# cvjena/ITAL

Measured on AMD Instinct MI355X. Metric: MI-scored candidates/sec per fetch_unlabelled(k) round, higher is better.
Workload: dtype f64; 1 GPU; USPS-shaped synthetic 9298x256, k=4, perfect user, full 2^t enumeration, fetch_unlabelled + update per step; n=9298, d=256, k=4, parallelism=candidate rows sharded over 1 GPU(s), 1 record all-gather per greedy step

## Files before the change

ital_amd/_lib.py:

```python
import ctypes
import os

HERE = os.path.dirname(os.path.abspath(__file__))
LIB_PATH = os.environ.get("ITAL_HIP_LIB", os.path.join(HERE, "libital_hip.so"))

c_void_p, c_int, c_int64, c_double = ctypes.c_void_p, ctypes.c_int, ctypes.c_int64, ctypes.c_double

ITAL_MAX_T = 8
ITAL_REC_HEADER = 10
ITAL_JUMP_BITS = 48
ITAL_GENERIC_MAX_DIM = 20
ITAL_GENERIC_MAX_REL = 16
ITAL_GENERIC_MAX_CALLS = 1 << 22
ITAL_TOPK_MAX = 4096
ITAL_ROUND_MAX_CAND = 1 << 21


class ItalBatch(ctypes.Structure):
    _fields_ = [("kmax", c_int), ("ldx", c_int), ("ldw", c_int), ("bidx", c_void_p), ("bgpos", c_void_p),
                ("bsort", c_void_p), ("bmu", c_void_p), ("sig", c_void_p), ("XB", c_void_p), ("XBn", c_void_p),
                ("VB", c_void_p)]


class ItalLabelBatch(ctypes.Structure):
# ... 264 lines not shown


ROWS_SIGNATURES = dict(
    [(name + "_t", _typed(SIGNATURES[name])) for name in
     ("ital_rbf_cols", "ital_cross_cov_cols", "ital_whiten_append", "ital_gp_append", "ital_score_step", "ital_fetch_round",
      "ital_select_local", "ital_select_fused", "ital_gather_block")] +
    [("ital_whiten_rows_t", _typed(REWHITEN_SIGNATURES["ital_whiten_rows"])),
     ("ital_ingest_rows_t", (c_int, [c_void_p, c_int, c_int64, c_int, c_int64, c_void_p, c_int, c_void_p, c_void_p, c_int64,
                                     c_void_p]))])


COMPACT_SIGNATURES = {
    "ital_compact_rows": (c_int, [c_void_p, c_void_p, c_int64, c_int, c_int, c_void_p, c_int64, c_void_p, c_void_p, c_void_p,
                                  c_void_p]),
    "ital_compact_cols": (c_int, [c_void_p, c_int64, c_int, c_void_p, c_void_p, c_int64, c_void_p, c_int64, c_void_p, c_int64,
                                  c_int, c_void_p, c_void_p, c_void_p, c_void_p]),
}


CTX_LIVE_SIGNATURES = {
    "ital_ctx_reserve": (c_int, [c_void_p, c_int, c_void_p]),
    "ital_ctx_add_rows": (c_int, [c_void_p, c_void_p, c_int64, c_int, c_void_p]),
    "ital_ctx_remove_rows": (c_int, [c_void_p, c_void_p, c_int64, c_void_p, c_void_p]),
    "ital_ctx_set_params": (c_int, [c_void_p, c_double, c_double, c_double, c_void_p]),
    "ital_ctx_evidence": (c_int, [c_void_p, c_void_p, c_int, c_void_p, c_void_p, c_void_p]),
}


COSINE_SIGNATURES = {
    "ital_cosine_min": (c_int, [c_void_p, c_int, c_void_p, c_int64, c_int, c_void_p, c_void_p, c_int, c_int, c_void_p, c_void_p]),
}


class ItalHipError(RuntimeError):
    pass


def load(path=LIB_PATH):
    if not os.path.exists(path):
        raise ImportError(
            f"{path} not found: build it with `python -m ital_amd.build` (hipcc, gfx950). "
            "ital_amd has no CPU fallback.")
    try:
        import torch
    except ImportError:
        pass
    lib = ctypes.CDLL(path)
    for name, (res, args) in list(SIGNATURES.items()) + list(CTX_SIGNATURES.items()) + list(DENSE_SIGNATURES.items()) + \
            list(ADAPT_SIGNATURES.items()) + list(REVOKE_SIGNATURES.items()) + list(REWHITEN_SIGNATURES.items()) + \
            list(EVIDENCE_SIGNATURES.items()) + list(INGEST_SIGNATURES.items()) + list(ROWS_SIGNATURES.items()) + \
            list(COMPACT_SIGNATURES.items()) + list(EVIDENCE_GRAD_SIGNATURES.items()) + list(LOO_GRAD_SIGNATURES.items()) + \
            list(CTX_LIVE_SIGNATURES.items()) + list(COSINE_SIGNATURES.items()) + list(INFLUENCE_SIGNATURES.items()) + \
            list(CTX_AUDIT_SIGNATURES.items()):
        fn = getattr(lib, name)
        fn.restype = res
        fn.argtypes = args
    return lib


_lib = None


def lib():
    global _lib
    if _lib is None:
        _lib = load()
    return _lib


def rows_fn(name, xtype):
    if xtype == INGEST_F64:
        return getattr(lib(), name)
    fn = getattr(lib(), name + "_t")
    return lambda *args: fn(*(args[:-1] + (xtype, args[-1])))


def check(rc):
    if rc != 0:
        raise ItalHipError(f"libital_hip: error {rc}: {lib().ital_last_error().decode()}")


def legacy_normals(n_skip, n_out, threads=1):
    import numpy as np
    n_skip, n_out = int(n_skip), int(n_out)
    state = np.random.get_state(legacy=True)
    if state[0] != "MT19937":
# ... 13 lines not shown
```

ital_amd/csrc/score.hip:

```cpp
#include <hip/hip_runtime.h>
#include <stdint.h>

#include <type_traits>

#include "device_math.h"
#include "ital_hip.h"
#include "ital_internal.h"
#include "ital_rows.h"
#include "qmc_common.h"
#include "qmc_exact.h"
#include "qmc_seed.h"
#include "qmc_share.h"
#include "select_common.h"

#ifndef ITAL_QMC_HOTK
#define ITAL_QMC_HOTK 1
#endif
#ifndef ITAL_QMC_MAIN_NH
#define ITAL_QMC_MAIN_NH(T) ((T) == 6 || (T) == 8 ? 2 : 3)
#endif
#ifndef ITAL_QMC_WAVES
#define ITAL_QMC_WAVES(T) ((T) <= 4 || (T) == 6 || (T) == 8 ? 4 : 3)
#endif
#ifndef ITAL_QMC_MAIN_PS
#define ITAL_QMC_MAIN_PS(T) ((T) >= 7)
#endif
#ifndef ITAL_QMC_MAIN_KE6
#define ITAL_QMC_MAIN_KE6(T) ((T) == 8)
#endif
#ifndef ITAL_QMC_MAIN_KEN
#define ITAL_QMC_MAIN_KEN(T) ((T) == 7 ? 2 : -1)
#endif
#ifndef ITAL_QMC_MAIN_KE
#define ITAL_QMC_MAIN_KE(T) 1
#endif
#ifndef ITAL_QMC_MAIN_KS
#define ITAL_QMC_MAIN_KS(T) 0
#endif
#ifndef ITAL_QMC_MAIN_CFL
#define ITAL_QMC_MAIN_CFL(T) ((T) >= 7)
#endif

#ifndef ITAL_QMC_SHARE_LAST
#define ITAL_QMC_SHARE_LAST 1
#endif
#ifndef ITAL_QMC_BATCH_DIV
#define ITAL_QMC_BATCH_DIV 1
#endif
#ifndef ITAL_QMC_BATCH_PHINV
#define ITAL_QMC_BATCH_PHINV(T) ((T) <= 4 ? 3 : 0)
#endif
#ifndef ITAL_QMC_BATCH_PHI
#define ITAL_QMC_BATCH_PHI(T) ((T) <= 4 ? 3 : 0)
#endif
#ifndef ITAL_QMC_SHARE_RECS
#define ITAL_QMC_SHARE_RECS 4
#endif
#ifndef ITAL_QMC_SHARE_VCF
#define ITAL_QMC_SHARE_VCF 3
#endif

namespace ital {

struct ScoreArgs {
    int t;
    int64_t n_cand;
    const int32_t* cand;
    const uint8_t* alive;
    const double* mu;
    const double* s2;
    const double* C;
    int64_t ldc;
    int64_t row_offset;
    int64_t pos_offset;
    const int64_t* gpos;
    ital_batch b;
    double noise, eps;
    int label_mode;
    double* mi;
    int seed[6];
    const long long* jump;
    const long long* jumppat;
    const double* vk;
    int* status;
    SelectTail sel;
};

__device__ __forceinline__ double log_eps(double p, double eps) { return log(p + eps); }

__device__ __forceinline__ void mi_accumulate(double& mi, double pr, double pu, double eps, int mode) {
    double cur = log_eps(pu, eps) - log_eps(pr, eps);
    if (mode == 1) {
// ... 76 lines not shown
        const int64_t pc = (int64_t)blockIdx.x * 32 + threadIdx.x;
        if (pc < a.n_cand && a.alive[pc]) {
            double mi = 0.0;
#pragma unroll
            for (int q = 0; q < 4; q++) mi_accumulate(mi, vals[0][4 * threadIdx.x + q], vals[1][4 * threadIdx.x + q], a.eps, a.label_mode);
            a.mi[pc] = mi;
            c.val = mi;
            c.pos = a.gpos ? a.gpos[pc] : a.pos_offset + pc;
            c.loc = pc;
        }
    }
    if (a.sel.enabled) {
        c = block_best(c, 0);
        select_tail(a.sel, c, blockIdx.x, gridDim.x, true, gridDim.x);
    }
}

template <int T>
struct Qmc {
    static constexpr int NDIM = T - 1;
    static constexpr int NP = NDIM < 10 ? NDIM : 10;
    static constexpr int PRIME = P_TAB[NP - 1];
    static constexpr int NCOV = T * (T + 1) / 2;
    static constexpr int NCOR = T * (T - 1) / 2;
    static constexpr int NPAT = 1 << T;
    static constexpr int NCALLS = 2 << T;
    static constexpr int LAT = 8 * NDIM * 2;
    static constexpr int LATP = 5 * NDIM;
    static constexpr int R_LIM = NCOR, R_META = NCOR + T, R_LAT = NCOR + T + 1;
    static constexpr int REC = R_LAT + LATP;
    static constexpr int SLAB_RAW = NCOV + 2 * T + NDIM;
    static constexpr int SLAB = SLAB_RAW | 1;
    static constexpr int PREP_THREADS = T <= 6 ? 256 : 128;
    static constexpr int NH = ITAL_QMC_MAIN_NH(T);
    static constexpr int BPHI = ITAL_QMC_BATCH_DIV && !ITAL_LATTICE_PHI_CF ? ITAL_QMC_BATCH_PHI(T) : 0;
    static constexpr int BINV = ITAL_QMC_BATCH_DIV ? ITAL_QMC_BATCH_PHINV(T) : 0;
    static constexpr int TAILQ = 128 * NH;
    static constexpr bool PS = ITAL_QMC_MAIN_PS(T), CFL = PS && ITAL_QMC_MAIN_CFL(T);
    static constexpr bool SHARE = ITAL_QMC_SHARE_LAST && ITAL_QMC_HOTK && ITAL_QMC_FLIP && !PS &&
                                  QmcRounds<T, NH>::NCL == 1 && ITAL_QMC_SHARE_RECS * QmcRounds<T, NH>::REST <= 64 &&
                                  NPAT % ITAL_QMC_SHARE_RECS == 0;
    static constexpr int RPW = SHARE ? ITAL_QMC_SHARE_RECS : 1;
    static constexpr int WAVE_DOUBLES = LAT + TAILQ + (CFL ? NCOR + T : 0) + (SHARE ? 64 + 2 * RPW + 6 : 0);
    typedef typename std::conditional<(CFL && ITAL_QMC_MAIN_KS(T)), HotKS,
                typename std::conditional<(ITAL_QMC_MAIN_KEN(T) >= 0), HotKEn<(ITAL_QMC_MAIN_KEN(T) >= 0 ? ITAL_QMC_MAIN_KEN(T) : 0)>,
                typename std::conditional<(ITAL_QMC_MAIN_KE6(T)), HotKE6,
                    typename std::conditional<(ITAL_QMC_MAIN_KE(T)), HotKE, HotK>::type>::type>::type>::type Coef;
    static constexpr int64_t CAND_DOUBLES = (int64_t)NPAT * (REC + 1) + 3;
};
constexpr long long META_EVAL = 1, META_PRIOR_ONE = 2, META_POST_ONE = 4;
constexpr long long META_EXACT = 8;

template <int T>
__device__ void rcswp(int p, int q, double* cov, double* lim, unsigned& infi) {
    double tmp = lim[p]; lim[p] = lim[q]; lim[q] = tmp;
    unsigned bp = (infi >> p) & 1u, bq = (infi >> q) & 1u;
    infi = (infi & ~((1u << p) | (1u << q))) | (bq << p) | (bp << q);
    tmp = cov[pidx(p, p)]; cov[pidx(p, p)] = cov[pidx(q, q)]; cov[pidx(q, q)] = tmp;
    for (int j = 0; j < p; j++) { tmp = cov[pidx(p, j)]; cov[pidx(p, j)] = cov[pidx(q, j)]; cov[pidx(q, j)] = tmp; }
    for (int i = p + 1; i < q; i++) { tmp = cov[pidx(i, p)]; cov[pidx(i, p)] = cov[pidx(q, i)]; cov[pidx(q, i)] = tmp; }
    for (int i = q + 1; i < T; i++) { tmp = cov[pidx(i, p)]; cov[pidx(i, p)] = cov[pidx(i, q)]; cov[pidx(i, q)] = tmp; }
}

template <int T>
__device__ bool covsrt(double* cov, double* lim, double* y, unsigned& infi) {
    const double SQTWPI = 2.506628274631001, EPS = 1e-10;
    bool ok = true;
    for (int i = 0; i < T; i++) {
        double dmin = 0, emin = 1, zmin = 0, cvdiag = 0;
        int jmin = i;
        for (int j = i; j < T; j++) {
            const double cjj = cov[pidx(j, j)];
            if (cjj > EPS) {
                const double sumsq = sqrt_pos(cjj);
                double sum = 0;
// ... 27 lines not shown
        } else {
            ok = false;
            y[i] = 0;
        }
    }
    return ok;
}

template <int T>
__device__ __forceinline__ int early_verdict(const double (&l)[T]) {
    const double thr = 37.0 + 9.0 * sqrt((double)(T - 1));
    bool all_full = true, any_empty = false;
#pragma unroll
    for (int a = 0; a < T; a++) {
        if (l[a] > thr) any_empty = true;
        if (!(l[a] < -thr)) all_full = false;
    }
    return any_empty ? 4 : (all_full ? 2 : 0);
}

__device__ __forceinline__ int64_t list_position(const ScoreArgs& a, int64_t p) { return a.gpos ? a.gpos[p] : a.pos_offset + p; }

__global__ __launch_bounds__(256) void qmc_seed_kernel(SeedArgs s) {
    qmc_seed_body(s, (int64_t)blockIdx.x * blockDim.x + threadIdx.x);
}

static SeedArgs seed_args(const ScoreArgs& a, int ncalls, int64_t slab_lo, int64_t slab_n, int* seeds) {
    SeedArgs s = {a.alive, a.gpos, a.pos_offset, a.b.bgpos, a.t - 1, {a.seed[0], a.seed[1], a.seed[2], a.seed[3], a.seed[4], a.seed[5]},
                  a.jump, ncalls, slab_lo, slab_n, seeds};
    return s;
}

template <int T>
__global__ __launch_bounds__(Qmc<T>::PREP_THREADS) void qmc_prep_kernel(ScoreArgs a, int64_t slab_lo, int64_t slab_n,
                                                                         const int* __restrict__ seeds,
                                                                         double* __restrict__ recs) {
    using Q = Qmc<T>;
    extern __shared__ double lds_all[];
    const int64_t i = (int64_t)blockIdx.x * blockDim.x + threadIdx.x;
    if (i >= slab_n) return;
    const int64_t p = slab_lo + i;
    if (!a.alive[p]) return;
    const int r = blockIdx.y;
    const int row = a.cand[p];
    double* rec = recs + ((int64_t)i * Q::NPAT + r) * Q::REC;

    double mean[T], Sg[T][T];
#pragma unroll
    for (int v = 0; v < T - 1; v++) {
        mean[v] = a.b.bmu[v];
#pragma unroll
        for (int j = 0; j < T - 1; j++) Sg[v][j] = a.b.sig[v * a.b.kmax + j];
        const double c = a.C[(int64_t)v * a.ldc + row];
        Sg[v][T - 1] = c;
        Sg[T - 1][v] = c;
    }
    mean[T - 1] = a.mu[row];
    Sg[T - 1][T - 1] = a.s2[row];
    double sd[T], own[T];
    long long meta = 0;
    {
        double Lc[T][T];
#pragma unroll
        for (int v = 0; v < T; v++)
#pragma unroll
            for (int j = 0; j <= v; j++) {
                double x = Sg[v][j] + (v == j ? a.noise : 0.0);
#pragma unroll
                for (int q = 0; q < j; q++) x -= Lc[v][q] * Lc[j][q];
                Lc[v][j] = (v == j) ? sqrt(x) : x / Lc[j][j];
// ... 73 lines not shown
            if (sat0) verdict = 4;
            else if (sat1) verdict = 2;
            else evaluate = true;
        }
    }
    if (verdict == 2) meta |= META_PRIOR_ONE;
    if (evaluate) {
        meta |= META_EVAL | ((long long)infi << 8);
        const unsigned fl = ITAL_QMC_FLIP ? infi : 0u;
        for (int v = 1; v < T; v++)
            for (int j = 0; j < v; j++)
                rec[v * (v - 1) / 2 + j] = (((fl >> v) ^ (fl >> j)) & 1u) ? -cov[pidx(v, j)] : cov[pidx(v, j)];
        for (int v = 0; v < T; v++) rec[Q::R_LIM + v] = ((fl >> v) & 1u) ? -lim[v] : lim[v];
        const int* sp = seeds + i * 6;
        MrgState sti = {sp[0], sp[1], sp[2], sp[3], sp[4], sp[5]};
        mrg_apply(sti, a.jumppat + (int64_t)r * 18);
        MrgStateF st = mrg_to_f(sti);
        for (int j = 0; j < Q::NDIM; j++) gen[j] = (double)j;
        unsigned int* shifts = reinterpret_cast<unsigned int*>(rec + Q::R_LAT);
        unsigned char* perm = reinterpret_cast<unsigned char*>(rec + Q::R_LAT + 4 * Q::NDIM);
        for (int sft = 0; sft < 8; sft++) {
            for (int j = 1; j <= Q::NDIM - 1; j++) {
                const double u = mrg_next_f(st);
                const int jp = (int)(j + u * (Q::NDIM + 1 - j));
                const double xt = gen[j - 1];
                gen[j - 1] = gen[jp - 1];
                gen[jp - 1] = xt;
            }
            for (int j = 0; j < Q::NDIM; j++) perm[sft * Q::NDIM + j] = (unsigned char)gen[j];
            for (int j = 0; j < Q::NDIM; j++) shifts[sft * Q::NDIM + j] = (unsigned int)mrg_next_z(st);
        }
    }
    rec[Q::R_META] = __longlong_as_double(meta);
}

template <int T>
__device__ __forceinline__ void qmc_main_shared(const uint8_t* __restrict__ alive, int64_t slab_lo, int64_t slab_n,
                                                const double* __restrict__ recs, const double* __restrict__ vk, double eps,
                                                int label_mode, double* __restrict__ terms) {
    using Q = Qmc<T>;
    using R = QmcRounds<T, Q::NH>;
    extern __shared__ double lds_all[];
    const int lane = threadIdx.x & 63;
    const int wid = __builtin_amdgcn_readfirstlane(threadIdx.x >> 6);
    const int64_t item0 = ((int64_t)blockIdx.x * 4 + wid) * Q::RPW;
    const int64_t i = item0 >> T;
    if (i >= slab_n) return;
    if (!alive[slab_lo + i]) return;
    double* lat = lds_all + (size_t)wid * Q::WAVE_DOUBLES;
    double* tailq = lat + Q::LAT;
    int first = -1;
    for (int j = Q::RPW - 1; j >= 0; j--)
        if (__double_as_longlong(uniform_f64(recs[(item0 + j) * Q::REC + Q::R_META])) & META_EVAL) first = j;
    double* lastv = tailq + Q::TAILQ;
    typename Q::Coef kk;
    kk.load();
    if (first >= 0) {
        const int j_own = lane >> 4;
        bool dead = j_own >= Q::RPW;
        if (!dead) dead = !(__double_as_longlong(recs[(item0 + j_own) * Q::REC + Q::R_META]) & META_EVAL);
        const double* rec = recs + (item0 + (dead ? first : j_own)) * Q::REC;
        const unsigned flips = (unsigned)(__double_as_longlong(rec[Q::R_META]) >> 8) & ((1u << T) - 1u);
        double cf[Q::NCOR > 0 ? Q::NCOR : 1], lm[T], xx[Q::NDIM > 0 ? Q::NDIM : 1];
#pragma unroll
        for (int q = 0; q < Q::NCOR; q++) cf[q] = rec[q];
#pragma unroll
        for (int q = 0; q < T; q++) lm[q] = rec[Q::R_LIM + q];
        const unsigned int* shifts = reinterpret_cast<const unsigned int*>(rec + Q::R_LAT);
        const unsigned char* perm = reinterpret_cast<const unsigned char*>(rec + Q::R_LAT + 4 * Q::NDIM);
        const int it = R::FULL * 64 * Q::NH + ((lane & 15) >> 1);
        const int sft = it / Q::PRIME;
        const int k = it - sft * Q::PRIME + 1;
#pragma unroll
        for (int j = 0; j < Q::NDIM; j++) {
            const int q = sft * Q::NDIM + j;
            const double gen = vk[perm[q]];
            const double shf = (double)shifts[q] * MRG_INVMP1 + (((flips >> (q % Q::NDIM)) & 1u) ? 0.5 : 0.0);
            const double v = k * gen + shf;
// ... 52 lines not shown
            const double part = qmc_lane_sum_full<T, typename Q::Coef, Q::NH, Q::BPHI, Q::BINV>(lat, w0, cf, lm, flips, tailq, ln, kk);
            __asm__ volatile("" : "+v"(jv));
            const int j2 = __builtin_amdgcn_readfirstlane(jv);
            const double acc = part + (ln < 16 ? lastv[16 * j2 + ln] : 0.0);
            pr = wave_sum(acc) / (16.0 * Q::PRIME);
#ifndef ITAL_NO_EXACT_FLAG
            if ((pr > 1.0 - EXACT_BAND || pr < EXACT_BAND) && ln == 0 && __double_as_longlong(keep[4]) != 0) {
                double* rm = reinterpret_cast<double*>(__double_as_longlong(keep[0])) + (__double_as_longlong(keep[5]) + j2) * Q::REC + Q::R_META;
                *rm = __longlong_as_double(__double_as_longlong(*rm) | META_EXACT);
            }
#endif
        }
        __asm__ volatile("" : "+v"(jv));
        if (ln == 0) lastv[64 + __builtin_amdgcn_readfirstlane(jv)] = pr;
        jv = jv + 1;
    }
    __builtin_amdgcn_fence(__ATOMIC_RELEASE, "wavefront");
    __builtin_amdgcn_wave_barrier();
    __builtin_amdgcn_fence(__ATOMIC_ACQUIRE, "wavefront");
    if (lane < Q::RPW) {
        const double* recs_k = reinterpret_cast<const double*>(__double_as_longlong(keep[0]));
        double* terms_k = reinterpret_cast<double*>(__double_as_longlong(keep[2]));
        const long long item_l = __double_as_longlong(keep[5]) + lane;
        const double eps_k = keep[3];
        const double pr_l = lastv[64 + lane];
        const long long meta_l = __double_as_longlong(recs_k[item_l * Q::REC + Q::R_META]);
        const double pu = (meta_l & META_POST_ONE) ? 1.0 : 0.0;
        const double cur = log_eps(pu, eps_k) - log_eps(pr_l, eps_k);
        terms_k[item_l] = __double_as_longlong(keep[4]) == 0 ? cur * pr_l : cur;
    }
}

template <int T>
__global__ __launch_bounds__(256) __attribute__((amdgpu_waves_per_eu(ITAL_QMC_WAVES(T), ITAL_QMC_WAVES(T)))) void qmc_main_kernel(
    const uint8_t* __restrict__ alive, int64_t slab_lo, int64_t slab_n, const double* __restrict__ recs,
    const double* __restrict__ vk, double eps, int label_mode, double* __restrict__ terms) {
    using Q = Qmc<T>;
    if constexpr (Q::SHARE) {
        qmc_main_shared<T>(alive, slab_lo, slab_n, recs, vk, eps, label_mode, terms);
        return;
    }
    extern __shared__ double lds_all[];
    const int lane = threadIdx.x & 63;
    const int wid = __builtin_amdgcn_readfirstlane(threadIdx.x >> 6);
    const int64_t item = (int64_t)blockIdx.x * 4 + wid;
    const int64_t i = item >> T;
    if (i >= slab_n) return;
    if (!alive[slab_lo + i]) return;
    const double* rec = recs + item * Q::REC;
    const long long meta = __double_as_longlong(uniform_f64(rec[Q::R_META]));
    double pr = (meta & META_PRIOR_ONE) ? 1.0 : 0.0;
    if (meta & META_EVAL) {
        double* lat = lds_all + (size_t)wid * Q::WAVE_DOUBLES;
        double* tailq = lat + Q::LAT;
        const unsigned flips = ITAL_QMC_FLIP ? (unsigned)(meta >> 8) & ((1u << T) - 1u) : 0u;
        {
            const unsigned int* shifts = reinterpret_cast<const unsigned int*>(rec + Q::R_LAT);
            const unsigned char* perm = reinterpret_cast<const unsigned char*>(rec + Q::R_LAT + 4 * Q::NDIM);
            for (int q = lane; q < 8 * Q::NDIM; q += 64) {
                lat[q] = vk[perm[q]];
                lat[8 * Q::NDIM + q] = (double)shifts[q] * MRG_INVMP1 + (((flips >> (q % Q::NDIM)) & 1u) ? 0.5 : 0.0);
            }
        }
        double cf[Q::NCOR > 0 ? Q::NCOR : 1], lm[T];
        double* slab = tailq + Q::TAILQ;
        if (Q::CFL) {
            for (int q = lane; q < Q::NCOR + T; q += 64) slab[q] = rec[q];
        } else {
#pragma unroll
            for (int q = 0; q < Q::NCOR; q++) cf[q] = uniform_f64(rec[q]);
#pragma unroll
            for (int q = 0; q < T; q++) lm[q] = uniform_f64(rec[Q::R_LIM + q]);
        }
        const unsigned infi = (unsigned)(meta >> 8) & ((1u << T) - 1u);
        __builtin_amdgcn_fence(__ATOMIC_RELEASE, "wavefront");
        __builtin_amdgcn_wave_barrier();
        __builtin_amdgcn_fence(__ATOMIC_ACQUIRE, "wavefront");
#if ITAL_QMC_HOTK
        typename Q::Coef kk;
        kk.load();
        constexpr bool FL = ITAL_QMC_FLIP != 0;
        const double acc = Q::PS ? qmc_lane_sum_ps<T, typename Q::Coef, Q::NH, Q::CFL, FL>(lat, cf, lm, slab, infi, tailq, lane, kk)
                                 : qmc_lane_sum<T, typename Q::Coef, Q::NH, FL, Q::BPHI, Q::BINV>(lat, cf, lm, infi, tailq, lane, kk);
#else
        const double acc = qmc_lane_sum<T, LitK, Q::NH, ITAL_QMC_FLIP != 0>(lat, cf, lm, infi, tailq, lane);
#endif
        pr = wave_sum(acc) / (16.0 * Q::PRIME);
#ifndef ITAL_NO_EXACT_FLAG
        if (label_mode != 0 && (pr > 1.0 - EXACT_BAND || pr < EXACT_BAND) && lane == 0)
            const_cast<double*>(rec)[Q::R_META] = __longlong_as_double(meta | META_EXACT);
#endif
    }
    if (lane == 0) {
        const double pu = (meta & META_POST_ONE) ? 1.0 : 0.0;
        const double cur = log_eps(pu, eps) - log_eps(pr, eps);
        terms[item] = label_mode == 0 ? cur * pr : cur;
    }
}

template <int T>
__global__ __launch_bounds__(64) void qmc_exact_kernel(const uint8_t* __restrict__ alive, int64_t slab_lo, int64_t slab_n,
                                                       const double* __restrict__ recs, const double* __restrict__ vk, double eps,
                                                       int label_mode, double* __restrict__ terms) {
    using Q = Qmc<T>;
    extern __shared__ double lds_all[];
    const int lane = threadIdx.x;
    const int64_t item = blockIdx.x;
    const int64_t i = item >> T;
    if (i >= slab_n || !alive[slab_lo + i]) return;
    const double* rec = recs + item * Q::REC;
    const long long meta = __double_as_longlong(uniform_f64(rec[Q::R_META]));
    if (!(meta & META_EXACT)) return;
    double* slab = lds_all;
    double* lat = slab + Q::NCOV + T;
    double* tailq = lat + Q::LAT;
    double* vals = tailq + 128;
    const unsigned infi = (unsigned)(meta >> 8) & ((1u << T) - 1u);
    const unsigned fl = ITAL_QMC_FLIP ? infi : 0u;
    for (int q = lane; q < Q::NCOV; q += 64) {
        int row = 0;
        while ((row + 1) * (row + 2) / 2 <= q) row++;
        const int col = q - row * (row + 1) / 2;
        double v = 0.0;
        if (col < row) {
            v = rec[row * (row - 1) / 2 + col];
            if (((fl >> row) ^ (fl >> col)) & 1u) v = -v;
        }
        slab[q] = v;
    }
// ... 17 lines not shown
    if (lane == 0) {
        const double pu = (meta & META_POST_ONE) ? 1.0 : 0.0;
        const double cur = log_eps(pu, eps) - log_eps(pr, eps);
        terms[item] = label_mode == 0 ? cur * pr : cur;
    }
}

__global__ __launch_bounds__(256) void qmc_combine_kernel(const double* __restrict__ terms, const uint8_t* __restrict__ alive,
                                                          int64_t slab_lo, int64_t slab_n, int npat, int label_mode,
                                                          double* __restrict__ mi, int64_t pos_offset,
                                                          const int64_t* __restrict__ gpos, SelectTail sel, int part0,
                                                          int nparts, int finishing) {
    const int64_t i = (int64_t)blockIdx.x * blockDim.x + threadIdx.x;
    const bool valid = i < slab_n && alive[slab_lo + i];
    double s = 0.0;
    if (valid) {
        for (int r = 0; r < npat; r++) {
            const double cur = terms[i * npat + r];
            if (label_mode == 1) { if (cur > s) s = cur; }
            else if (label_mode == 2) { if (s == 0 || cur < s) s = cur; }
            else s += cur;
        }
        mi[slab_lo + i] = s;
    }
    if (sel.enabled) {
        const int64_t p = slab_lo + i;
        Best c = {s, valid ? (gpos ? gpos[p] : pos_offset + p) : -1, p};
        c = block_best(c, 0);
        select_tail(sel, c, part0 + blockIdx.x, nparts, finishing != 0, gridDim.x);
    }
}

template <int T>
static int launch_qmc(const ScoreArgs& a, double* work, int64_t work_doubles, int64_t sel_parts_len, hipEvent_t ev0, hipEvent_t ev1,
                      hipStream_t stream, bool seeds_ready, SeedArgs* seeds_only) {
    using Q = Qmc<T>;
    int64_t slab = work_doubles / Q::CAND_DOUBLES;
    if (slab < 1) return ital_fail(-12, "ital_score_step: workspace smaller than one candidate (see ital_score_workspace)");
    if (slab > a.n_cand) slab = a.n_cand;
    const size_t lds_main = (size_t)4 * Q::WAVE_DOUBLES * sizeof(double);
    const size_t lds_prep = (size_t)Q::PREP_THREADS * Q::SLAB * sizeof(double);
    static ItalLdsFlags lds_flags;
    if (lds_prep > 48 * 1024) {
        const int rc = ital_raise_lds_limit(reinterpret_cast<const void*>(&qmc_prep_kernel<T>), (int)lds_prep, lds_flags,
                                            "ital_score_step");
        if (rc) return rc;
    }
    double* recs = work;
    double* terms = recs + slab * Q::NPAT * Q::REC;
    int* seeds = reinterpret_cast<int*>(terms + slab * Q::NPAT);
    if (seeds_only) {
        if (slab < a.n_cand) return 1;
        *seeds_only = seed_args(a, Q::NCALLS, 0, a.n_cand, seeds);
        return 0;
    }
    int nparts = 0, part0 = 0;
    for (int64_t lo = 0; lo < a.n_cand; lo += slab) nparts += (int)(((a.n_cand - lo < slab ? a.n_cand - lo : slab) + 255) / 256);
    if (a.sel.enabled && 3 * (int64_t)nparts > sel_parts_len)
        return ital_fail(-22, "ital_score_step: sel_parts too small for the blocks of this step");
    for (int64_t lo = 0; lo < a.n_cand; lo += slab) {
        const int64_t n = a.n_cand - lo < slab ? a.n_cand - lo : slab;
        if (!(seeds_ready && slab >= a.n_cand))
            ITAL_LAUNCH(qmc_seed_kernel, dim3((unsigned)((n + 255) / 256)), dim3(256), 0, stream, seed_args(a, Q::NCALLS, lo, n, seeds));
        ITAL_LAUNCH(qmc_prep_kernel<T>, dim3((unsigned)((n + Q::PREP_THREADS - 1) / Q::PREP_THREADS), Q::NPAT),
                           dim3(Q::PREP_THREADS), lds_prep, stream, a, lo, n, seeds, recs);
        if (ev0 && lo == 0) (void)hipEventRecord(ev0, stream);
        ITAL_LAUNCH(qmc_main_kernel<T>, dim3((unsigned)((n * Q::NPAT + 4 * Q::RPW - 1) / (4 * Q::RPW))), dim3(256), lds_main, stream, a.alive, lo,
                           n, recs, a.vk, a.eps, a.label_mode, terms);
        if (ev1 && lo + n >= a.n_cand) (void)hipEventRecord(ev1, stream);
        if (a.label_mode != 0) {
            const size_t lds_x = (size_t)(Q::NCOV + T + Q::LAT + 128 + 16 * Q::PRIME) * sizeof(double);
            static ItalLdsFlags lds_xflags;
            if (lds_x > 48 * 1024) {
                const int rc = ital_raise_lds_limit(reinterpret_cast<const void*>(&qmc_exact_kernel<T>), (int)lds_x, lds_xflags, "ital_score_step");
                if (rc) return rc;
            }
            ITAL_LAUNCH(qmc_exact_kernel<T>, dim3((unsigned)(n * Q::NPAT)), dim3(64), lds_x, stream, a.alive, lo, n, recs, a.vk, a.eps,
                        a.label_mode, terms);
        }
        ITAL_LAUNCH(qmc_combine_kernel, dim3((unsigned)((n + 255) / 256)), dim3(256), 0, stream, terms, a.alive, lo, n,
                    Q::NPAT, a.label_mode, a.mi, a.pos_offset, a.gpos, a.sel, part0, nparts, lo + n >= a.n_cand ? 1 : 0);
        part0 += (int)((n + 255) / 256);
        int rc = ital_check_launch("ital_score_step(qmc)");
        if (rc) return rc;
    }
    return 0;
}

template <int T>
static int64_t qmc_cand_doubles() { return Qmc<T>::CAND_DOUBLES; }

static int64_t cand_doubles(int t) {
    switch (t) {
        case 3: return qmc_cand_doubles<3>();
        case 4: return qmc_cand_doubles<4>();
        case 5: return qmc_cand_doubles<5>();
        case 6: return qmc_cand_doubles<6>();
        case 7: return qmc_cand_doubles<7>();
        case 8: return qmc_cand_doubles<8>();
    }
    return 0;
}

}

using namespace ital;

extern "C" int64_t ital_score_workspace(int t, int64_t n_cand) {
    if (t < 3 || t > ITAL_MAX_T || n_cand <= 0) return 0;
    return cand_doubles(t) * n_cand;
}

extern "C" int ital_record_len(int ldx, int ldw, int kmax) {
    if (ldx < 0 || ldw < 0 || kmax < 0) return 0;
    return ITAL_REC_HEADER + ldx + ldw + kmax;
}

extern "C" int64_t ital_round_workspace(int k, int64_t n_cand, int64_t cap_doubles) {
    if (k > ITAL_MAX_T) k = ITAL_MAX_T;
    const int64_t one_slab = ital_score_workspace(k, n_cand > 0 ? n_cand : 1);
    if (one_slab == 0) return 0;
    int64_t cap = cap_doubles > 0 ? cap_doubles : one_slab;
    const int64_t least = ital_score_workspace(k, 1);
    if (cap < least) cap = least;
    return one_slab < cap ? one_slab : cap;
}

extern "C" int64_t ital_sel_parts_len(int k, int64_t n_cand, int64_t work_doubles) {
    if (n_cand < 0) n_cand = 0;
    if (k > ITAL_MAX_T) k = ITAL_MAX_T;
    int64_t slabs = 0;
    if (k >= 3 && n_cand > 0) {
        const int64_t per = ital_score_workspace(k, 1);
        const int64_t fit = work_doubles / per;
        slabs = fit >= n_cand ? 1 : (fit < 1 ? n_cand : (n_cand + fit - 1) / fit);
    }
    return 3 * (n_cand / 32 + 64 + slabs);
}

int ital_score_step_internal(const ital_score_desc* d, int xtype, hipStream_t stream, bool seeds_ready, ital::SeedArgs* seeds_only) {
    if (!d) return ital_fail(-22, "ital_score_step: null descriptor");
    if (seeds_only && (d->n_cand <= 0 || d->t < 3 || d->t > ITAL_MAX_T || !d->work || !d->jump)) return 1;
    if (d->n_cand <= 0) return 0;
    if (d->t < 1 || d->t > ITAL_MAX_T) return ital_fail(-22, "ital_score_step: batch dimension outside 1..ITAL_MAX_T");
// ... 60 lines not shown
```

Baseline: 16.51 million candidates/s.

## Split QMC main-kernel tail wave into fine-grained single-record work items

Computes device wave slots from occupancy and CU count, then plans the main QMC launch so that the last partial wave of candidates is handled by per-record (non-shared) waves instead of shared multi-record waves. The intent is to reduce tail-wave imbalance, where a few shared-record waves run alone at the end of the kernel. The cost is a runtime occupancy query (cached per device), an extra branch in the kernel, and the single-record path being less efficient per record.

Measured after the change: 16.67 million candidates/s (median of 6 runs). No clear change (+1.0%).

```diff
diff --git a/include/ital_qmc_launch.h b/include/ital_qmc_launch.h
--- /dev/null
+++ b/include/ital_qmc_launch.h
@@ -0,0 +1,18 @@
+#ifndef ITAL_QMC_LAUNCH_H
+#define ITAL_QMC_LAUNCH_H
+
+#include <stdint.h>
+
+#ifdef __cplusplus
+extern "C" {
+#endif
+
+int ital_qmc_launch_plan(int t, int64_t n_cand, int64_t slots, int64_t* n_big, int64_t* blocks);
+
+void ital_qmc_set_slots(int64_t waves);
+
+#ifdef __cplusplus
+}
+#endif
+
+#endif
diff --git a/ital_amd/_lib.py b/ital_amd/_lib.py
--- a/ital_amd/_lib.py
+++ b/ital_amd/_lib.py
@@ -320,6 +320,12 @@
 }
 
 
+QMC_LAUNCH_SIGNATURES = {
+    "ital_qmc_launch_plan": (c_int, [c_int, c_int64, c_int64, ctypes.POINTER(c_int64), ctypes.POINTER(c_int64)]),
+    "ital_qmc_set_slots": (None, [c_int64]),
+}
+
+
 class ItalHipError(RuntimeError):
     pass
 
@@ -339,7 +345,7 @@
             list(EVIDENCE_SIGNATURES.items()) + list(INGEST_SIGNATURES.items()) + list(ROWS_SIGNATURES.items()) + \
             list(COMPACT_SIGNATURES.items()) + list(EVIDENCE_GRAD_SIGNATURES.items()) + list(LOO_GRAD_SIGNATURES.items()) + \
             list(CTX_LIVE_SIGNATURES.items()) + list(COSINE_SIGNATURES.items()) + list(INFLUENCE_SIGNATURES.items()) + \
-            list(CTX_AUDIT_SIGNATURES.items()):
+            list(CTX_AUDIT_SIGNATURES.items()) + list(QMC_LAUNCH_SIGNATURES.items()):
         fn = getattr(lib, name)
         fn.restype = res
         fn.argtypes = args
diff --git a/ital_amd/csrc/score.hip b/ital_amd/csrc/score.hip
--- a/ital_amd/csrc/score.hip
+++ b/ital_amd/csrc/score.hip
@@ -1,11 +1,13 @@
 #include <hip/hip_runtime.h>
 #include <stdint.h>
 
+#include <atomic>
 #include <type_traits>
 
 #include "device_math.h"
 #include "ital_hip.h"
 #include "ital_internal.h"
+#include "ital_qmc_launch.h"
 #include "ital_rows.h"
 #include "qmc_common.h"
 #include "qmc_exact.h"
@@ -58,6 +60,15 @@
 #endif
 #ifndef ITAL_QMC_SHARE_VCF
 #define ITAL_QMC_SHARE_VCF 3
+#endif
+#ifndef ITAL_QMC_MAIN_WPB
+#define ITAL_QMC_MAIN_WPB(T) 4
+#endif
+#ifndef ITAL_QMC_FINE_TAIL
+#define ITAL_QMC_FINE_TAIL 1
+#endif
+#ifndef ITAL_QMC_FINE_DEN
+#define ITAL_QMC_FINE_DEN 4
 #endif
 
 namespace ital {
@@ -209,6 +220,8 @@
                                   QmcRounds<T, NH>::NCL == 1 && ITAL_QMC_SHARE_RECS * QmcRounds<T, NH>::REST <= 64 &&
                                   NPAT % ITAL_QMC_SHARE_RECS == 0;
     static constexpr int RPW = SHARE ? ITAL_QMC_SHARE_RECS : 1;
+    static constexpr int WPB = ITAL_QMC_MAIN_WPB(T);
+    static constexpr bool FINE = SHARE && ITAL_QMC_FINE_TAIL;
     static constexpr int WAVE_DOUBLES = LAT + TAILQ + (CFL ? NCOR + T : 0) + (SHARE ? 64 + 2 * RPW + 6 : 0);
     typedef typename std::conditional<(CFL && ITAL_QMC_MAIN_KS(T)), HotKS,
                 typename std::conditional<(ITAL_QMC_MAIN_KEN(T) >= 0), HotKEn<(ITAL_QMC_MAIN_KEN(T) >= 0 ? ITAL_QMC_MAIN_KEN(T) : 0)>,
@@ -456,7 +469,7 @@
     extern __shared__ double lds_all[];
     const int lane = threadIdx.x & 63;
     const int wid = __builtin_amdgcn_readfirstlane(threadIdx.x >> 6);
-    const int64_t item0 = ((int64_t)blockIdx.x * 4 + wid) * Q::RPW;
+    const int64_t item0 = ((int64_t)blockIdx.x * Q::WPB + wid) * Q::RPW;
     const int64_t i = item0 >> T;
     if (i >= slab_n) return;
     if (!alive[slab_lo + i]) return;
@@ -575,18 +588,12 @@
 }
 
 template <int T>
-__global__ __launch_bounds__(256) __attribute__((amdgpu_waves_per_eu(ITAL_QMC_WAVES(T), ITAL_QMC_WAVES(T)))) void qmc_main_kernel(
-    const uint8_t* __restrict__ alive, int64_t slab_lo, int64_t slab_n, const double* __restrict__ recs,
-    const double* __restrict__ vk, double eps, int label_mode, double* __restrict__ terms) {
+__device__ __forceinline__ void qmc_main_single(int64_t item, int wid, const uint8_t* __restrict__ alive, int64_t slab_lo,
+                                                int64_t slab_n, const double* __restrict__ recs, const double* __restrict__ vk,
+                                                double eps, int label_mode, double* __restrict__ terms) {
     using Q = Qmc<T>;
-    if constexpr (Q::SHARE) {
-        qmc_main_shared<T>(alive, slab_lo, slab_n, recs, vk, eps, label_mode, terms);
-        return;
-    }
     extern __shared__ double lds_all[];
     const int lane = threadIdx.x & 63;
-    const int wid = __builtin_amdgcn_readfirstlane(threadIdx.x >> 6);
-    const int64_t item = (int64_t)blockIdx.x * 4 + wid;
     const int64_t i = item >> T;
     if (i >= slab_n) return;
     if (!alive[slab_lo + i]) return;
@@ -638,6 +645,30 @@
         const double pu = (meta & META_POST_ONE) ? 1.0 : 0.0;
         const double cur = log_eps(pu, eps) - log_eps(pr, eps);
         terms[item] = label_mode == 0 ? cur * pr : cur;
+    }
+}
+
+template <int T>
+__global__ __launch_bounds__(64 * ITAL_QMC_MAIN_WPB(T)) __attribute__((amdgpu_waves_per_eu(ITAL_QMC_WAVES(T), ITAL_QMC_WAVES(T))))
+void qmc_main_kernel(const uint8_t* __restrict__ alive, int64_t slab_lo, int64_t slab_n, int64_t n_big,
+                     const double* __restrict__ recs, const double* __restrict__ vk, double eps, int label_mode,
+                     double* __restrict__ terms) {
+    using Q = Qmc<T>;
+    const int wid = __builtin_amdgcn_readfirstlane(threadIdx.x >> 6);
+    if constexpr (Q::SHARE) {
+        if constexpr (Q::FINE) {
+            const int64_t b_big = (n_big * (Q::NPAT / Q::RPW) + Q::WPB - 1) / Q::WPB;
+            if ((int64_t)blockIdx.x >= b_big) {
+                const int64_t item = n_big * Q::NPAT + ((int64_t)blockIdx.x - b_big) * Q::WPB + wid;
+                qmc_main_single<T>(item, wid, alive, slab_lo, slab_n, recs, vk, eps, label_mode, terms);
+                return;
+            }
+            qmc_main_shared<T>(alive, slab_lo, n_big, recs, vk, eps, label_mode, terms);
+        } else {
+            qmc_main_shared<T>(alive, slab_lo, slab_n, recs, vk, eps, label_mode, terms);
+        }
+    } else {
+        qmc_main_single<T>((int64_t)blockIdx.x * Q::WPB + wid, wid, alive, slab_lo, slab_n, recs, vk, eps, label_mode, terms);
     }
 }
 
@@ -721,13 +752,50 @@
 }
 
 template <int T>
+static void qmc_plan(int64_t n, int64_t slots, int64_t* n_big, int64_t* blocks) {
+    using Q = Qmc<T>;
+    constexpr int64_t WPC = Q::NPAT / Q::RPW;
+    int64_t nb = n;
+    if (Q::FINE && slots > 0 && n * WPC >= slots) {
+        const int64_t rem = (n * WPC) % slots;
+        const int64_t n_fine = (rem + WPC - 1) / WPC;
+        if (rem > 0 && n_fine * WPC * ITAL_QMC_FINE_DEN <= slots && n_fine * Q::NPAT <= slots) nb = n - n_fine;
+    }
+    *n_big = nb;
+    *blocks = (nb * WPC + Q::WPB - 1) / Q::WPB + ((n - nb) * Q::NPAT + Q::WPB - 1) / Q::WPB;
+}
+
+static std::atomic<int64_t> g_qmc_slots{0};
+
+template <int T>
+static int64_t qmc_slots(size_t lds_main) {
+    const int64_t forced = g_qmc_slots.load(std::memory_order_relaxed);
+    if (forced > 0) return forced;
+    static std::atomic<int64_t> cached[16];
+    int dev = 0;
+    if (hipGetDevice(&dev) != hipSuccess || dev < 0 || dev >= 16) return 0;
+    int64_t s = cached[dev].load(std::memory_order_relaxed);
+    if (s == 0) {
+        int per_cu = 0, cus = 0;
+        s = -1;
+        if (hipOccupancyMaxActiveBlocksPerMultiprocessor(&per_cu, qmc_main_kernel<T>, 64 * Qmc<T>::WPB, lds_main) == hipSuccess &&
+            hipDeviceGetAttribute(&cus, hipDeviceAttributeMultiprocessorCount, dev) == hipSuccess && per_cu > 0 && cus > 0)
+            s = (int64_t)per_cu * cus * Qmc<T>::WPB;
+        else
+            (void)hipGetLastError();
+        cached[dev].store(s, std::memory_order_relaxed);
+    }
+    return s > 0 ? s : 0;
+}
+
+template <int T>
 static int launch_qmc(const ScoreArgs& a, double* work, int64_t work_doubles, int64_t sel_parts_len, hipEvent_t ev0, hipEvent_t ev1,
                       hipStream_t stream, bool seeds_ready, SeedArgs* seeds_only) {
     using Q = Qmc<T>;
     int64_t slab = work_doubles / Q::CAND_DOUBLES;
     if (slab < 1) return ital_fail(-12, "ital_score_step: workspace smaller than one candidate (see ital_score_workspace)");
     if (slab > a.n_cand) slab = a.n_cand;
-    const size_t lds_main = (size_t)4 * Q::WAVE_DOUBLES * sizeof(double);
+    const size_t lds_main = (size_t)Q::WPB * Q::WAVE_DOUBLES * sizeof(double);
     const size_t lds_prep = (size_t)Q::PREP_THREADS * Q::SLAB * sizeof(double);
     static ItalLdsFlags lds_flags;
     if (lds_prep > 48 * 1024) {
@@ -754,8 +822,10 @@
         ITAL_LAUNCH(qmc_prep_kernel<T>, dim3((unsigned)((n + Q::PREP_THREADS - 1) / Q::PREP_THREADS), Q::NPAT),
                            dim3(Q::PREP_THREADS), lds_prep, stream, a, lo, n, seeds, recs);
         if (ev0 && lo == 0) (void)hipEventRecord(ev0, stream);
-        ITAL_LAUNCH(qmc_main_kernel<T>, dim3((unsigned)((n * Q::NPAT + 4 * Q::RPW - 1) / (4 * Q::RPW))), dim3(256), lds_main, stream, a.alive, lo,
-                           n, recs, a.vk, a.eps, a.label_mode, terms);
+        int64_t n_big, blocks;
+        qmc_plan<T>(n, Q::FINE ? qmc_slots<T>(lds_main) : 0, &n_big, &blocks);
+        ITAL_LAUNCH(qmc_main_kernel<T>, dim3((unsigned)blocks), dim3(64 * Q::WPB), lds_main, stream, a.alive, lo, n, n_big, recs, a.vk,
+                    a.eps, a.label_mode, terms);
         if (ev1 && lo + n >= a.n_cand) (void)hipEventRecord(ev1, stream);
         if (a.label_mode != 0) {
             const size_t lds_x = (size_t)(Q::NCOV + T + Q::LAT + 128 + 16 * Q::PRIME) * sizeof(double);
@@ -799,6 +869,22 @@
     if (t < 3 || t > ITAL_MAX_T || n_cand <= 0) return 0;
     return cand_doubles(t) * n_cand;
 }
+
+extern "C" int ital_qmc_launch_plan(int t, int64_t n_cand, int64_t slots, int64_t* n_big, int64_t* blocks) {
+    if (t < 3 || t > ITAL_MAX_T || n_cand <= 0 || slots < 0 || !n_big || !blocks)
+        return ital_fail(-22, "ital_qmc_launch_plan: t outside 3..ITAL_MAX_T, no candidates, negative slots or a null pointer");
+    switch (t) {
+        case 3: qmc_plan<3>(n_cand, slots, n_big, blocks); break;
+        case 4: qmc_plan<4>(n_cand, slots, n_big, blocks); break;
+        case 5: qmc_plan<5>(n_cand, slots, n_big, blocks); break;
+        case 6: qmc_plan<6>(n_cand, slots, n_big, blocks); break;
+        case 7: qmc_plan<7>(n_cand, slots, n_big, blocks); break;
+        case 8: qmc_plan<8>(n_cand, slots, n_big, blocks); break;
+    }
+    return 0;
+}
+
+extern "C" void ital_qmc_set_slots(int64_t waves) { g_qmc_slots.store(waves > 0 ? waves : 0, std::memory_order_relaxed); }
 
 extern "C" int ital_record_len(int ldx, int ldw, int kmax) {
     if (ldx < 0 || ldw < 0 || kmax < 0) return 0;
```

## Group prep kernel per candidate block, stage records in LDS, split lattice replay lanes

Applied to the files above, without the earlier changes.

For small t (T<=4), the QMC prep kernel now handles all 2^T patterns of a group of candidates in one block instead of a grid with one y-slice per pattern. Each record is built in LDS and then written out with coalesced double2 stores. A second half of the block (replay lanes) generates the lattice permutations and shifts in parallel with the covariance sort and update-meta work. The sort and swap run fully in registers with static indexing. The aim is to cut the scattered per-thread record writes, the dynamic local-memory indexing and the serial per-thread work in prep. The cost is more LDS per block, duplicated candidate loads across lanes, and a constrained occupancy hint.

Result: no change. 16.35 million candidates/s before, 16.42 million candidates/s after (median of 2 runs) (+0.4%).

```diff
diff --git a/ital_amd/csrc/score.hip b/ital_amd/csrc/score.hip
--- a/ital_amd/csrc/score.hip
+++ b/ital_amd/csrc/score.hip
@@ -52,6 +52,15 @@
 #endif
 #ifndef ITAL_QMC_BATCH_PHI
 #define ITAL_QMC_BATCH_PHI(T) ((T) <= 4 ? 3 : 0)
+#endif
+#ifndef ITAL_QMC_PREP_GROUP
+#define ITAL_QMC_PREP_GROUP 1
+#endif
+#ifndef ITAL_QMC_PREP_GROUP_RECS
+#define ITAL_QMC_PREP_GROUP_RECS 256
+#endif
+#ifndef ITAL_QMC_PREP_REPLAY
+#define ITAL_QMC_PREP_REPLAY 1
 #endif
 #ifndef ITAL_QMC_SHARE_RECS
 #define ITAL_QMC_SHARE_RECS 4
@@ -200,6 +209,12 @@
     static constexpr int SLAB_RAW = NCOV + 2 * T + NDIM;
     static constexpr int SLAB = SLAB_RAW | 1;
     static constexpr int PREP_THREADS = T <= 6 ? 256 : 128;
+    static constexpr bool GROUPED = ITAL_QMC_PREP_GROUP && T <= 4;
+    static constexpr int GROUP_RECS = ITAL_QMC_PREP_GROUP_RECS;
+    static constexpr int GROUP = GROUP_RECS >> (T <= 4 ? T : 4);
+    static constexpr int GROUP_THREADS = ITAL_QMC_PREP_REPLAY ? 2 * GROUP_RECS : GROUP_RECS;
+    static constexpr int GROUP_WAVES_MIN = GROUPED && ITAL_QMC_PREP_REPLAY ? 6 : 1;
+    static constexpr int GROUP_WAVES_MAX = GROUPED && ITAL_QMC_PREP_REPLAY ? 6 : 8;
     static constexpr int NH = ITAL_QMC_MAIN_NH(T);
     static constexpr int BPHI = ITAL_QMC_BATCH_DIV && !ITAL_LATTICE_PHI_CF ? ITAL_QMC_BATCH_PHI(T) : 0;
     static constexpr int BINV = ITAL_QMC_BATCH_DIV ? ITAL_QMC_BATCH_PHINV(T) : 0;
@@ -302,10 +317,79 @@
 }
 
 template <int T>
-__global__ __launch_bounds__(Qmc<T>::PREP_THREADS) void qmc_prep_kernel(ScoreArgs a, int64_t slab_lo, int64_t slab_n,
-                                                                         const int* __restrict__ seeds,
-                                                                         double* __restrict__ recs) {
+__device__ __forceinline__ void prep_candidate(const ScoreArgs& a, int row, double (&mean)[T], double (&Sg)[T][T]) {
+#pragma unroll
+    for (int v = 0; v < T - 1; v++) {
+        mean[v] = a.b.bmu[v];
+#pragma unroll
+        for (int j = 0; j < T - 1; j++) Sg[v][j] = a.b.sig[v * a.b.kmax + j];
+        const double c = a.C[(int64_t)v * a.ldc + row];
+        Sg[v][T - 1] = c;
+        Sg[T - 1][v] = c;
+    }
+    mean[T - 1] = a.mu[row];
+    Sg[T - 1][T - 1] = a.s2[row];
+}
+
+template <int T>
+__device__ __forceinline__ long long prep_update_meta(const ScoreArgs& a, int r, const double (&mean)[T], const double (&Sg)[T][T]) {
+    double Lc[T][T];
+#pragma unroll
+    for (int v = 0; v < T; v++)
+#pragma unroll
+        for (int j = 0; j <= v; j++) {
+            double x = Sg[v][j] + (v == j ? a.noise : 0.0);
+#pragma unroll
+            for (int q = 0; q < j; q++) x -= Lc[v][q] * Lc[j][q];
+            Lc[v][j] = (v == j) ? sqrt(x) : x / Lc[j][j];
+        }
+    double Li[T][T];
+#pragma unroll
+    for (int j = 0; j < T; j++) {
+#pragma unroll
+        for (int v = 0; v < T; v++) {
+            if (v < j) { Li[v][j] = 0; continue; }
+            double x = (v == j) ? 1.0 : 0.0;
+#pragma unroll
+            for (int q = j; q < v; q++) x -= Lc[v][q] * Li[q][j];
+            Li[v][j] = x / Lc[v][v];
+        }
+    }
+    double own[T];
+#pragma unroll
+    for (int v = 0; v < T; v++) {
+        double mu_u = mean[v], gvv = 0;
+#pragma unroll
+        for (int j = 0; j < T; j++) {
+            double w = 0;
+#pragma unroll
+            for (int q = (v > j ? v : j); q < T; q++) w += Li[q][v] * Li[q][j];
+            const double gvj = (v == j ? 1.0 : 0.0) - a.noise * w;
+            const double f = ((r >> (T - 1 - j)) & 1) ? 1.0 : -1.0;
+            mu_u += gvj * (f - mean[j]);
+            if (j == v) gvv = gvj;
+        }
+        const double lim_u = -mu_u / sqrt(a.noise * gvv);
+        own[v] = ((r >> (T - 1 - v)) & 1) ? lim_u : -lim_u;
+    }
+    const int e = early_verdict<T>(own);
+    if (e == 0) atomicOr(a.status, 4);
+    return e == 2 ? META_POST_ONE : 0;
+}
+
+template <int T>
+__device__ __forceinline__ void qmc_prep_grouped(const ScoreArgs& a, int64_t slab_lo, int64_t slab_n, const int* __restrict__ seeds,
+                                                 double* __restrict__ recs);
+
+template <int T>
+__global__ __launch_bounds__(Qmc<T>::GROUPED ? Qmc<T>::GROUP_THREADS : Qmc<T>::PREP_THREADS) __attribute__((amdgpu_waves_per_eu(
+    Qmc<T>::GROUP_WAVES_MIN, Qmc<T>::GROUP_WAVES_MAX))) void qmc_prep_kernel(
+    ScoreArgs a, int64_t slab_lo, int64_t slab_n, const int* __restrict__ seeds, double* __restrict__ recs) {
     using Q = Qmc<T>;
+    if constexpr (Q::GROUPED) {
+        qmc_prep_grouped<T>(a, slab_lo, slab_n, seeds, recs);
+        return;
+    }
     extern __shared__ double lds_all[];
     const int64_t i = (int64_t)blockIdx.x * blockDim.x + threadIdx.x;
     if (i >= slab_n) return;
@@ -445,6 +529,233 @@
         }
     }
     rec[Q::R_META] = __longlong_as_double(meta);
+}
+
+template <int T>
+__device__ __forceinline__ void rcswp_static(int p, int q, double (&cov)[T * (T + 1) / 2], double (&lim)[T], unsigned& infi) {
+    double tmp = lim[p]; lim[p] = lim[q]; lim[q] = tmp;
+    unsigned bp = (infi >> p) & 1u, bq = (infi >> q) & 1u;
+    infi = (infi & ~((1u << p) | (1u << q))) | (bq << p) | (bp << q);
+    tmp = cov[pidx(p, p)]; cov[pidx(p, p)] = cov[pidx(q, q)]; cov[pidx(q, q)] = tmp;
+#pragma unroll
+    for (int j = 0; j < T; j++)
+        if (j < p) { tmp = cov[pidx(p, j)]; cov[pidx(p, j)] = cov[pidx(q, j)]; cov[pidx(q, j)] = tmp; }
+#pragma unroll
+    for (int i = 0; i < T; i++)
+        if (i > p && i < q) { tmp = cov[pidx(i, p)]; cov[pidx(i, p)] = cov[pidx(q, i)]; cov[pidx(q, i)] = tmp; }
+#pragma unroll
+    for (int i = 0; i < T; i++)
+        if (i > q) { tmp = cov[pidx(i, p)]; cov[pidx(i, p)] = cov[pidx(i, q)]; cov[pidx(i, q)] = tmp; }
+}
+
+template <int T>
+__device__ __forceinline__ bool covsrt_reg(double (&cov)[T * (T + 1) / 2], double (&lim)[T], double (&y)[T], unsigned& infi) {
+    const double SQTWPI = 2.506628274631001, EPS = 1e-10;
+    bool ok = true;
+#pragma unroll
+    for (int i = 0; i < T; i++) {
+        double dmin = 0, emin = 1, zmin = 0, cvdiag = 0;
+        int jmin = i;
+#pragma unroll
+        for (int j = i; j < T; j++) {
+            const double cjj = cov[pidx(j, j)];
+            if (cjj > EPS) {
+                const double sumsq = sqrt_pos(cjj);
+                double sum = 0;
+#pragma unroll
+                for (int k = 0; k < i; k++) sum += cov[pidx(j, k)] * y[k];
+                const double z = fast_div(lim[j] - sum, sumsq);
+                const double ph = mvn_phi(z);
+                const bool lower = (infi >> j) & 1u;
+                const double d = lower ? ph : 0.0;
+                const double e = lower ? 1.0 : fmax(ph, 0.0);
+                if (emin + d >= e + dmin) { jmin = j; zmin = z; dmin = d; emin = e; cvdiag = sumsq; }
+            }
+        }
+#pragma unroll
+        for (int q = i + 1; q < T; q++)
+            if (jmin == q) rcswp_static<T>(i, q, cov, lim, infi);
+        cov[pidx(i, i)] = cvdiag;
+        if (cvdiag > 0) {
+            const double rdiag = fast_div(1.0, cvdiag);
+#pragma unroll
+            for (int l = i + 1; l < T; l++) {
+                cov[pidx(l, i)] = cov[pidx(l, i)] * rdiag;
+#pragma unroll
+                for (int j = i + 1; j <= l; j++) cov[pidx(l, j)] -= cov[pidx(l, i)] * cov[pidx(j, i)];
+            }
+            const bool lower = (infi >> i) & 1u;
+            if (emin > dmin + EPS) {
+                const double dens = -exp_neg(-zmin * zmin / 2) * (1.0 / SQTWPI);
+                const double yl = lower ? dens : 0.0, yu = lower ? 0.0 : dens;
+                y[i] = fast_div(yu - yl, emin - dmin);
+            } else {
+                y[i] = zmin;
+            }
+#pragma unroll
+            for (int j = 0; j <= i; j++) cov[pidx(i, j)] = cov[pidx(i, j)] * rdiag;
+            lim[i] = lim[i] * rdiag;
+        } else {
+            ok = false;
+            y[i] = 0;
+        }
+    }
+    return ok;
+}
+
+template <int T>
+__device__ __forceinline__ unsigned prep_prior_limits(int r, const double (&mean)[T], const double (&Sg)[T][T], double (&sd)[T],
+                                                      double (&lim)[T], double (&own)[T]) {
+    unsigned infi = 0;
+#pragma unroll
+    for (int v = 0; v < T; v++) {
+        sd[v] = sqrt(Sg[v][v]);
+        const double piv = -mean[v] / sd[v];
+        const unsigned bit = (r >> (T - 1 - v)) & 1;
+        lim[v] = piv;
+        own[v] = bit ? piv : -piv;
+        infi |= bit << v;
+    }
+    return infi;
+}
+
+template <int T>
+__device__ __forceinline__ void prep_lattice(const ScoreArgs& a, const int* __restrict__ sp, int r, double* lat) {
+    using Q = Qmc<T>;
+    MrgState sti = {sp[0], sp[1], sp[2], sp[3], sp[4], sp[5]};
+    mrg_apply(sti, a.jumppat + (int64_t)r * 18);
+    MrgStateF st = mrg_to_f(sti);
+    unsigned gen[Q::NDIM], pw[2 * Q::NDIM];
+#pragma unroll
+    for (int j = 0; j < Q::NDIM; j++) gen[j] = (unsigned)j;
+#pragma unroll
+    for (int w = 0; w < 2 * Q::NDIM; w++) pw[w] = 0u;
+    unsigned int* shifts = reinterpret_cast<unsigned int*>(lat);
+    unsigned int* perm = reinterpret_cast<unsigned int*>(lat + 4 * Q::NDIM);
+#pragma unroll
+    for (int sft = 0; sft < 8; sft++) {
+#pragma unroll
+        for (int j = 1; j <= Q::NDIM - 1; j++) {
+            const double u = mrg_next_f(st);
+            const int jp = (int)(j + u * (Q::NDIM + 1 - j));
+            const unsigned xt = gen[j - 1];
+            unsigned other = xt;
+#pragma unroll
+            for (int c = j; c < Q::NDIM; c++)
+                if (jp - 1 == c) { other = gen[c]; gen[c] = xt; }
+            gen[j - 1] = other;
+        }
+#pragma unroll
+        for (int j = 0; j < Q::NDIM; j++) {
+            const int q = sft * Q::NDIM + j;
+            pw[q >> 2] |= gen[j] << (8 * (q & 3));
+        }
+#pragma unroll
+        for (int j = 0; j < Q::NDIM; j++) shifts[sft * Q::NDIM + j] = (unsigned int)mrg_next_z(st);
+    }
+#pragma unroll
+    for (int w = 0; w < 2 * Q::NDIM; w++) perm[w] = pw[w];
+}
+
+template <int T>
+__device__ __forceinline__ void qmc_prep_grouped(const ScoreArgs& a, int64_t slab_lo, int64_t slab_n, const int* __restrict__ seeds,
+                                                 double* __restrict__ recs) {
+    using Q = Qmc<T>;
+    extern __shared__ __attribute__((aligned(16))) double prep_stage[];
+    const int tid = threadIdx.x & (Q::GROUP_RECS - 1);
+    const bool replay_lanes = ITAL_QMC_PREP_REPLAY && threadIdx.x >= Q::GROUP_RECS;
+    const int64_t i = (int64_t)blockIdx.x * Q::GROUP + (tid >> T);
+    const int r = tid & (Q::NPAT - 1);
+    const bool live = i < slab_n && a.alive[slab_lo + (i < slab_n ? i : 0)];
+    double* rec = prep_stage + tid * Q::REC;
+    if (live) {
+        const int row = a.cand[slab_lo + i];
+        double mean[T], Sg[T][T];
+        prep_candidate<T>(a, row, mean, Sg);
+        double sd[T], lim[T], own[T];
+        unsigned infi = prep_prior_limits<T>(r, mean, Sg, sd, lim, own);
+        int verdict = early_verdict<T>(own);
+        if (ITAL_QMC_PREP_REPLAY ? replay_lanes : true) {
+            if (verdict == 0) {
+                prep_lattice<T>(a, seeds + i * 6, r, rec + Q::R_LAT);
+            } else {
+#pragma unroll
+                for (int q = 0; q < Q::LATP; q++) rec[Q::R_LAT + q] = 0.0;
+            }
+        }
+        if (!replay_lanes) {
+            long long meta = prep_update_meta<T>(a, r, mean, Sg);
+            double cf[Q::NCOR], lm[T];
+#pragma unroll
+            for (int q = 0; q < Q::NCOR; q++) cf[q] = 0.0;
+#pragma unroll
+            for (int q = 0; q < T; q++) lm[q] = 0.0;
+            if (verdict == 0) {
+                double cov[Q::NCOV], y[T];
+#pragma unroll
+                for (int v = 0; v < T; v++) {
+#pragma unroll
+                    for (int j = 0; j < v; j++) cov[pidx(v, j)] = Sg[v][j] / (sd[v] * sd[j]);
+                    cov[pidx(v, v)] = 1.0;
+                }
+                const bool okc = covsrt_reg<T>(cov, lim, y, infi);
+                if (!okc) {
+                    atomicOr(a.status, 2);
+                } else {
+                    bool sat1 = true, sat0 = false;
+#pragma unroll
+                    for (int v = 0; v < T; v++) {
+                        double bound = 0;
+#pragma unroll
+                        for (int j = 0; j < v; j++) bound += fabs(cov[pidx(v, j)]) * 9.0;
+                        const bool lower = (infi >> v) & 1u;
+                        if (lower) {
+                            if (!(lim[v] + bound < -37.0)) sat1 = false;
+                            if (lim[v] - bound > 37.0) sat0 = true;
+                        } else {
+                            if (!(lim[v] - bound > 37.0)) sat1 = false;
+                            if (lim[v] + bound < -37.0) sat0 = true;
+                        }
+                    }
+                    if (sat0) verdict = 4;
+                    else if (sat1) verdict = 2;
+                    else {
+                        meta |= META_EVAL | ((long long)infi << 8);
+                        const unsigned fl = ITAL_QMC_FLIP ? infi : 0u;
+#pragma unroll
+                        for (int v = 1; v < T; v++)
+#pragma unroll
+                            for (int j = 0; j < v; j++)
+                                cf[v * (v - 1) / 2 + j] = (((fl >> v) ^ (fl >> j)) & 1u) ? -cov[pidx(v, j)] : cov[pidx(v, j)];
+#pragma unroll
+                        for (int v = 0; v < T; v++) lm[v] = ((fl >> v) & 1u) ? -lim[v] : lim[v];
+                    }
+                }
+            }
+            if (verdict == 2) meta |= META_PRIOR_ONE;
+#pragma unroll
+            for (int q = 0; q < Q::NCOR; q++) rec[q] = cf[q];
+#pragma unroll
+            for (int q = 0; q < T; q++) rec[Q::R_LIM + q] = lm[q];
+            rec[Q::R_META] = __longlong_as_double(meta);
+        }
+    }
+    __syncthreads();
+    constexpr int CAND_CHUNKS = Q::NPAT * Q::REC / 2;
+    static_assert(Q::NPAT * Q::REC % 2 == 0 && Q::GROUP * Q::NPAT == Q::GROUP_RECS, "prep group layout");
+    double* out = recs + (int64_t)blockIdx.x * Q::GROUP_RECS * Q::REC;
+    const bool wide = (reinterpret_cast<uintptr_t>(recs) & 15) == 0;
+    for (int c = threadIdx.x; c < Q::GROUP * CAND_CHUNKS; c += Q::GROUP_THREADS) {
+        const int64_t ic = (int64_t)blockIdx.x * Q::GROUP + c / CAND_CHUNKS;
+        if (ic >= slab_n || !a.alive[slab_lo + ic]) continue;
+        const double2 v = *reinterpret_cast<const double2*>(prep_stage + 2 * c);
+        if (wide) {
+            *reinterpret_cast<double2*>(out + 2 * c) = v;
+        } else {
+            out[2 * c] = v.x;
+            out[2 * c + 1] = v.y;
+        }
+    }
 }
 
 template <int T>
@@ -728,7 +1039,10 @@
     if (slab < 1) return ital_fail(-12, "ital_score_step: workspace smaller than one candidate (see ital_score_workspace)");
     if (slab > a.n_cand) slab = a.n_cand;
     const size_t lds_main = (size_t)4 * Q::WAVE_DOUBLES * sizeof(double);
-    const size_t lds_prep = (size_t)Q::PREP_THREADS * Q::SLAB * sizeof(double);
+    const size_t lds_prep = Q::GROUPED ? (size_t)Q::GROUP_RECS * Q::REC * sizeof(double)
+                                       : (size_t)Q::PREP_THREADS * Q::SLAB * sizeof(double);
+    const int prep_threads = Q::GROUPED ? Q::GROUP_THREADS : Q::PREP_THREADS, prep_cands = Q::GROUPED ? Q::GROUP : Q::PREP_THREADS;
+    const unsigned prep_grid_y = Q::GROUPED ? 1 : Q::NPAT;
     static ItalLdsFlags lds_flags;
     if (lds_prep > 48 * 1024) {
         const int rc = ital_raise_lds_limit(reinterpret_cast<const void*>(&qmc_prep_kernel<T>), (int)lds_prep, lds_flags,
@@ -751,8 +1065,8 @@
         const int64_t n = a.n_cand - lo < slab ? a.n_cand - lo : slab;
         if (!(seeds_ready && slab >= a.n_cand))
             ITAL_LAUNCH(qmc_seed_kernel, dim3((unsigned)((n + 255) / 256)), dim3(256), 0, stream, seed_args(a, Q::NCALLS, lo, n, seeds));
-        ITAL_LAUNCH(qmc_prep_kernel<T>, dim3((unsigned)((n + Q::PREP_THREADS - 1) / Q::PREP_THREADS), Q::NPAT),
-                           dim3(Q::PREP_THREADS), lds_prep, stream, a, lo, n, seeds, recs);
+        ITAL_LAUNCH(qmc_prep_kernel<T>, dim3((unsigned)((n + prep_cands - 1) / prep_cands), prep_grid_y),
+                           dim3(prep_threads), lds_prep, stream, a, lo, n, seeds, recs);
         if (ev0 && lo == 0) (void)hipEventRecord(ev0, stream);
         ITAL_LAUNCH(qmc_main_kernel<T>, dim3((unsigned)((n * Q::NPAT + 4 * Q::RPW - 1) / (4 * Q::RPW))), dim3(256), lds_main, stream, a.alive, lo,
                            n, recs, a.vk, a.eps, a.label_mode, terms);
```
